# leimao/Voice-Converter-CycleGAN

Measured on NVIDIA H100. Metric: CycleGAN-VC train steps/sec @ batch 256x[24,128] MCEP, higher is better.
Workload: dtype f16f8 (forward / data gradient: fp16 MMA + two e4m3 cross-term MMAs = 2 MMA units per product; weight gradient: fp16 MMA alone, 1 unit; f32 accumulate)

## Files before the change

voice-converter-cyclegan_b200/csrc/tc_gemm.cu:

```cuda
#include "tc_gemm.cuh"
#include "geom.h"
#include "kernels.cuh"
#include "wgmma.cuh"

#include <cuda.h>
#include <stdint.h>
#include <stdio.h>

namespace {

typedef CUresult (*EncodeTiledFn)(CUtensorMap*, CUtensorMapDataType, cuuint32_t, void*, const cuuint64_t*, const cuuint64_t*,
                                  const cuuint32_t*, const cuuint32_t*, CUtensorMapInterleave, CUtensorMapSwizzle,
                                  CUtensorMapL2promotion, CUtensorMapFloatOOBfill);
EncodeTiledFn get_encoder() {
  static EncodeTiledFn fn = nullptr;
  if (!fn) {
    void* p = nullptr; cudaDriverEntryPointQueryResult q;
    if (cudaGetDriverEntryPoint("cuTensorMapEncodeTiled", &p, cudaEnableDefault, &q) == cudaSuccess && q == cudaDriverEntryPointSuccess)
      fn = (EncodeTiledFn)p;
  }
  return fn;
}
bool make_tmap3(CUtensorMap* m, const void* base, uint64_t d0, uint64_t d1, uint64_t d2, uint32_t b1) {
  EncodeTiledFn enc = get_encoder();
  if (!enc) return false;
  cuuint64_t dims[3] = {d0, d1, d2};
  cuuint64_t strides[2] = {d0 * 2, d0 * d1 * 2};
  cuuint32_t box[3] = {64, b1, 1};
  cuuint32_t es[3] = {1, 1, 1};
  return enc(m, CU_TENSOR_MAP_DATA_TYPE_BFLOAT16, 3, const_cast<void*>(base), dims, strides, box, es, CU_TENSOR_MAP_INTERLEAVE_NONE,
             CU_TENSOR_MAP_SWIZZLE_128B, CU_TENSOR_MAP_L2_PROMOTION_L2_256B, CU_TENSOR_MAP_FLOAT_OOB_FILL_NONE) == CUDA_SUCCESS;
}

bool make_tmap3_t(CUtensorMap* m, const void* base, CUtensorMapDataType dt, int esize, uint64_t d0, uint64_t d1, uint64_t d2, uint32_t b0, uint32_t b1) {
  EncodeTiledFn enc = get_encoder();
  if (!enc) return false;
  cuuint64_t dims[3] = {d0, d1, d2};
  cuuint64_t strides[2] = {d0 * (uint64_t)esize, d0 * d1 * (uint64_t)esize};
  cuuint32_t box[3] = {b0, b1, 1};
  cuuint32_t es[3] = {1, 1, 1};
  return enc(m, dt, 3, const_cast<void*>(base), dims, strides, box, es, CU_TENSOR_MAP_INTERLEAVE_NONE,
             b0 * esize == 64 ? CU_TENSOR_MAP_SWIZZLE_64B : CU_TENSOR_MAP_SWIZZLE_128B, CU_TENSOR_MAP_L2_PROMOTION_L2_256B,
             CU_TENSOR_MAP_FLOAT_OOB_FILL_NONE) == CUDA_SUCCESS;
}

__device__ __forceinline__ uint32_t smem_u32(const void* p) { return (uint32_t)__cvta_generic_to_shared(p); }

__device__ __forceinline__ void mbar_init(uint64_t* bar, uint32_t count) {
  asm volatile("mbarrier.init.shared::cta.b64 [%0], %1;" ::"r"(smem_u32(bar)), "r"(count));
}
__device__ __forceinline__ void fence_barrier_init() { asm volatile("fence.mbarrier_init.release.cluster;" ::: "memory"); }
__device__ __forceinline__ void mbar_wait(uint64_t* bar, uint32_t parity) {
  asm volatile(
      "{\n\t"
      ".reg .pred p;\n\t"
      "WAIT_LOOP:\n\t"
      "mbarrier.try_wait.parity.shared::cta.b64 p, [%0], %1;\n\t"
      "@p bra.uni WAIT_DONE;\n\t"
      "bra.uni WAIT_LOOP;\n\t"
      "WAIT_DONE:\n\t"
      "}" ::"r"(smem_u32(bar)), "r"(parity) : "memory");
}
__device__ __forceinline__ void cp_async16(uint32_t dst_smem, const void* src, uint32_t src_bytes) {
  asm volatile("cp.async.cg.shared.global [%0], [%1], 16, %2;" ::"r"(dst_smem), "l"(src), "r"(src_bytes) : "memory");
}
__device__ __forceinline__ void cp_async_arrive_noinc(uint64_t* bar) {
  asm volatile("cp.async.mbarrier.arrive.noinc.shared::cta.b64 [%0];" ::"r"(smem_u32(bar)) : "memory");
}
__device__ __forceinline__ void mbar_expect_tx(uint64_t* bar, uint32_t bytes) {
  asm volatile("mbarrier.arrive.expect_tx.shared::cta.b64 _, [%0], %1;" ::"r"(smem_u32(bar)), "r"(bytes) : "memory");
}
__device__ __forceinline__ void tma_load3(uint32_t dst_smem, const CUtensorMap* map, int c0, int c1, int c2, uint64_t* bar) {
  asm volatile("cp.async.bulk.tensor.3d.shared::cluster.global.tile.mbarrier::complete_tx::bytes [%0], [%1, {%2, %3, %4}], [%5];"
               ::"r"(dst_smem), "l"(map), "r"(c0), "r"(c1), "r"(c2), "r"(smem_u32(bar)) : "memory");
}
__device__ __forceinline__ void tma_prefetch_desc(const CUtensorMap* map) {
  asm volatile("prefetch.tensormap [%0];" ::"l"(map) : "memory");
}
__device__ __forceinline__ void fence_proxy_async() { asm volatile("fence.proxy.async.shared::cta;" ::: "memory"); }
__device__ __forceinline__ uint64_t make_desc(uint32_t smem_addr, uint32_t lbo_bytes, uint32_t sbo_bytes, uint64_t layout = 1) {
  return (uint64_t)((smem_addr >> 4) & 0x3FFF) | ((uint64_t)((lbo_bytes >> 4) & 0x3FFF) << 16) |
         ((uint64_t)((sbo_bytes >> 4) & 0x3FFF) << 32) | (layout << 62);
}
__device__ __forceinline__ uint64_t make_desc64(uint32_t smem_addr) { return make_desc(smem_addr, 16, 512, 2); }
template <int N>
__device__ __forceinline__ void fence_acc(float (&d)[N]) {
#pragma unroll
  for (int i = 0; i < N; ++i) asm volatile("" : "+f"(d[i])::"memory");
}
__device__ __forceinline__ void mbar_arrive(uint64_t* bar) {
  asm volatile("mbarrier.arrive.shared::cta.b64 _, [%0];" ::"r"(smem_u32(bar)) : "memory");
}
__device__ __forceinline__ void consumer_bar() { asm volatile("bar.sync 3, 256;" ::: "memory"); }
__device__ __forceinline__ void st_shared16(uint32_t addr, uint4 v) {
  asm volatile("st.shared.v4.b32 [%0], {%1, %2, %3, %4};" ::"r"(addr), "r"(v.x), "r"(v.y), "r"(v.z), "r"(v.w) : "memory");
}
__device__ __forceinline__ uint4 e4m3x8_to_f16x8(uint2 v) {
  uint32_t w[4];
#pragma unroll
  for (int i = 0; i < 4; ++i) {
    const uint32_t src = (i < 2 ? v.x : v.y) >> (16 * (i & 1));
    const __half2_raw h = __nv_cvt_fp8x2_to_halfraw2((__nv_fp8x2_storage_t)(src & 0xFFFFu), __NV_E4M3);
    w[i] = (uint32_t)h.x | ((uint32_t)h.y << 16);
  }
  return make_uint4(w[0], w[1], w[2], w[3]);
}

struct FastDiv { uint32_t mul, shr, d; };
__host__ inline FastDiv make_fastdiv(uint32_t d) {
  FastDiv f; f.d = d;
  uint32_t l = 0; while ((1ull << l) < d) ++l;
  f.mul = (uint32_t)(((1ull << 32) * ((1ull << l) - d)) / d + 1);
  f.shr = l;
  return f;
}
__device__ __forceinline__ uint32_t fdiv(uint32_t n, const FastDiv& f) { return (uint32_t)(((uint64_t)__umulhi(n, f.mul) + n) >> f.shr); }

__device__ __forceinline__ uint32_t sw128(int r, int c) { return (uint32_t)((r >> 3) * 1024 + (r & 7) * 128 + ((c ^ (r & 7)) << 4)); }

struct TcNTParams {
  GatherGeom g;
  const __nv_bfloat16 *a_hi, *a_lo; int a_ld; int C;
  const __nv_bfloat16 *b_hi, *b_lo; int Nw;
  int N;
  int n_tiles;
  int debug;
  float* dst; int d_ld; const float* bias; int accumulate;
  int perm; int Cc;
  int R;
  const float *gamma_a, *beta_a, *gamma_g, *beta_g;
  float* stats;
  const float* resid;
  float* y; __nv_bfloat16 *y_hi, *y_lo;
  int C_out;
  const float* bp; int bp_ld;
  __nv_bfloat16 *dp_hi, *dp_lo; int dp_ld;
  float *dbeta_a, *dgamma_a, *dbeta_g, *dgamma_g;
  CUtensorMap tm_b_hi, tm_b_lo;
  const uint8_t *a8_hi, *a8_lo;
  CUtensorMap tm_b8_hi, tm_b8_lo;
  uint8_t* y8;
  PackGeom pk;
  FastDiv div_bw, div_w;
};

struct RowPos { int b, y, x; };
__device__ __forceinline__ RowPos nt_row(const TcNTParams& p, long long m) {
  RowPos r;
  r.y = (int)fdiv((uint32_t)m, p.div_bw);
  const uint32_t rem = (uint32_t)m - (uint32_t)r.y * p.div_bw.d;
  r.b = (int)fdiv(rem, p.div_w);
  r.x = (int)(rem - (uint32_t)r.b * p.div_w.d);
  return r;
}
__device__ __forceinline__ uint32_t nt_tile_taps(const TcNTParams& p, long long m0, long long M) {
  const long long m1 = m0 + 127 < M ? m0 + 127 : M - 1;
  return gather_tap_mask(p.g, nt_row(p, m0).y, nt_row(p, m1).y);
}

struct TcTNParams {
  GatherGeom g;
  const __nv_bfloat16 *x_hi, *x_lo; int x_ld; int C;
  const __nv_bfloat16 *g_hi, *g_lo; int g_ld; int N;
  float* dw_a; float* dw_g; int n_split;
  int ksplit;
  FastDiv div_hw, div_w;
  CUtensorMap tm_g_hi, tm_g_lo;
  const uint8_t *x8_hi, *x8_lo;
  const uint8_t *g8_hi, *g8_lo;
  int w16;
  int fold_n;
  float* part; long long part_k, numel_a;
};

__device__ __forceinline__ float* tn_dst(float* base, int slab, int C, int c, int ncols, int col, int fold_n) {
  if (fold_n) { const int t = col / fold_n; return base + ((long long)t * C + c) * fold_n + (col - t * fold_n); }
  return base + ((long long)slab * C + c) * ncols + col;
}

constexpr int kProducerThreads = 128;


template <int BN, int NPL>
struct NTCfg {
  static constexpr int A_PLANE = 128 * 128;
  static constexpr int B_PLANE = BN * 128;
  static constexpr int PLANES = NPL == 2 ? 2 : 1;
  static constexpr int STAGE = PLANES * (A_PLANE + B_PLANE);
  static constexpr int STAGES = (192 * 1024) / STAGE;
  static constexpr int SMEM = STAGES * STAGE + 1024;
  static_assert(STAGES * STAGE >= 128 * BN * 4, "the finished fp32 tile is staged over the pipeline stages");
};

template <int BN>
__device__ __forceinline__ int acc_off(int r, int n) { return r * BN + (n & ~31) + ((((n >> 2) & 7) ^ (r & 7)) << 2) + (n & 3); }
template <int BN>
__device__ __forceinline__ void acc_ld32(const float* acc, int r, int col, uint32_t (&v)[32]) {
#pragma unroll
  for (int c = 0; c < 8; ++c) {
    const float4 x = *reinterpret_cast<const float4*>(acc + r * BN + col + ((c ^ (r & 7)) << 2));
    v[4 * c] = __float_as_uint(x.x); v[4 * c + 1] = __float_as_uint(x.y); v[4 * c + 2] = __float_as_uint(x.z); v[4 * c + 3] = __float_as_uint(x.w);
  }
}

__device__ __forceinline__ float warp_colsum32(float (&t)[32], int lane) {
#pragma unroll
  for (int o = 16, n = 32; o >= 1; o >>= 1, n >>= 1) {
    const bool up = (lane & o) != 0;
#pragma unroll
    for (int i = 0; i < n / 2; ++i) {
      float send = up ? t[i] : t[i + n / 2];
      float keep = up ? t[i + n / 2] : t[i];
      t[i] = keep + __shfl_xor_sync(0xffffffffu, send, o);
    }
  }
  return t[0];
}
__device__ __forceinline__ void epi_bar(int id) { asm volatile("bar.sync %0, 128;" ::"r"(id) : "memory"); }

__device__ __forceinline__ float sample_sum(float v, float (*xch)[32], int q, int lane, int spw, int barid) {
  if (spw == 1) return v;
  epi_bar(barid);
  xch[q][lane] = v;
  epi_bar(barid);
  const int q0 = (q / spw) * spw;
  float r = 0.f;
  for (int w = 0; w < spw; ++w) r += xch[q0 + w][lane];
  return r;
}
__device__ __forceinline__ void bc4(const float* p, float (&v)[4]) { const float4 x = *reinterpret_cast<const float4*>(p); v[0] = x.x; v[1] = x.y; v[2] = x.z; v[3] = x.w; }
__device__ __forceinline__ float fast_sigmoid(float x) { return __fdividef(1.f, 1.f + __expf(-x)); }
__device__ __forceinline__ void chunk_norm_coeffs(const float (&v)[32], const float* __restrict__ gamma, const float* __restrict__ beta,
                                                  int ch, int R, float (*xch)[32], float* bc, int q, int lane, int spw, int barid, float& mean, float& rstd) {
  float t[32];
#pragma unroll
  for (int k = 0; k < 32; ++k) t[k] = v[k];
  float s = warp_colsum32(t, lane);
  s = sample_sum(s, xch, q, lane, spw, barid);
  mean = s / (float)R;
  __syncwarp();
  bc[lane] = mean;
  __syncwarp();
#pragma unroll
  for (int k = 0; k < 32; k += 4) {
    float4 m4 = *reinterpret_cast<const float4*>(bc + k);
    float d0 = v[k] - m4.x, d1 = v[k + 1] - m4.y, d2 = v[k + 2] - m4.z, d3 = v[k + 3] - m4.w;
    t[k] = d0 * d0; t[k + 1] = d1 * d1; t[k + 2] = d2 * d2; t[k + 3] = d3 * d3;
  }
  float ss = warp_colsum32(t, lane);
  ss = sample_sum(ss, xch, q, lane, spw, barid);
  rstd = 1.f / sqrtf(ss / (float)R + 1e-6f);
  const float sc = rstd * gamma[ch + lane];
  const float of = beta[ch + lane] - mean * sc;
  __syncwarp();
  bc[lane] = sc; bc[32 + lane] = of;
  __syncwarp();
}

__device__ __forceinline__ void pair_norm_coeffs(const float (&v0)[32], const float (&v1)[32], const float* __restrict__ gamma, const float* __restrict__ beta,
                                                 int ch, int R, float (*xch)[32], float* bc, int q, int lane, int spw, int barid, float& mean, float& rstd) {
  float t[32];
#pragma unroll
  for (int k = 0; k < 32; ++k) t[k] = v0[k] + v1[k];
  float s = warp_colsum32(t, lane);
  s = sample_sum(s, xch, q, lane, spw, barid);
  const float inv = 1.f / (float)(2 * R);
  mean = s * inv;
  __syncwarp();
  bc[lane] = mean;
  __syncwarp();
#pragma unroll
  for (int k = 0; k < 32; k += 4) {
    float4 m4 = *reinterpret_cast<const float4*>(bc + k);
    const float m[4] = {m4.x, m4.y, m4.z, m4.w};
#pragma unroll
    for (int j = 0; j < 4; ++j) { const float d0 = v0[k + j] - m[j], d1 = v1[k + j] - m[j]; t[k + j] = fmaf(d0, d0, d1 * d1); }
  }
  float ss = warp_colsum32(t, lane);
  ss = sample_sum(ss, xch, q, lane, spw, barid);
  rstd = 1.f / sqrtf(ss * inv + 1e-6f);
  const float sc = rstd * gamma[ch + lane];
  const float of = beta[ch + lane] - mean * sc;
  __syncwarp();
  bc[lane] = sc; bc[32 + lane] = of;
  __syncwarp();
}

__device__ __forceinline__ uint32_t hp_off(int r, int c) { return (uint32_t)(r * 16 + ((c ^ ((r >> 1) & 3)) << 2)); }
template <class F>
__device__ __forceinline__ void rows_out(float* stg, const float (&o)[32], int lane, F f) {
  const int hc = lane & 3, hr = lane >> 2;
#pragma unroll
  for (int h = 0; h < 2; ++h) {
    __syncwarp();
#pragma unroll
    for (int c = 0; c < 4; ++c)
      *reinterpret_cast<float4*>(stg + hp_off(lane, c)) = make_float4(o[16 * h + 4 * c], o[16 * h + 4 * c + 1], o[16 * h + 4 * c + 2], o[16 * h + 4 * c + 3]);
    __syncwarp();
#pragma unroll
    for (int i = 0; i < 4; ++i) {
      const int rr = hr + 8 * i;
      f(rr, 16 * h + 4 * hc, *reinterpret_cast<const float4*>(stg + hp_off(rr, hc)));
    }
  }
}
__device__ __forceinline__ void rows_in(float* stg, float (&v)[32], int lane, const float4 (&pre)[8]) {
  const int hc = lane & 3, hr = lane >> 2;
#pragma unroll
  for (int h = 0; h < 2; ++h) {
    __syncwarp();
#pragma unroll
    for (int i = 0; i < 4; ++i) *reinterpret_cast<float4*>(stg + hp_off(hr + 8 * i, hc)) = pre[4 * h + i];
    __syncwarp();
#pragma unroll
    for (int c = 0; c < 4; ++c) {
      const float4 x = *reinterpret_cast<const float4*>(stg + hp_off(lane, c));
      v[16 * h + 4 * c] = x.x; v[16 * h + 4 * c + 1] = x.y; v[16 * h + 4 * c + 2] = x.z; v[16 * h + 4 * c + 3] = x.w;
    }
  }
}
__device__ __forceinline__ void rows_fetch(float4 (&pre)[8], const float* base, long long ld, long long mq, long long M, int col, int lane) {
  const int hc = lane & 3, hr = lane >> 2;
#pragma unroll
  for (int h = 0; h < 2; ++h)
// ... 598 lines not shown
  static constexpr int SMEM = STAGES * STAGE + 1024;
};

template <int NPL, int W16, int DET>
__global__ void __launch_bounds__(kNTThreads, 1)
tc_gg_tn_kernel(const __grid_constant__ TcTNParams p) {
  static_assert(W16 == 0 || NPL == 3, "the fp16-only weight gradient is a form of CGVC_PREC_F16F8");
  using Cfg = TNCfg<NPL, W16>;
  constexpr int S = Cfg::STAGES;
  constexpr int BN = 256;
  extern __shared__ uint8_t smem_raw[];
  __shared__ __align__(8) uint64_t full_bar[S], empty_bar[S];

  const uint32_t smem_base = (smem_u32(smem_raw) + 1023u) & ~1023u;
  const int warp = threadIdx.x >> 5, lane = threadIdx.x & 31;
  const GatherGeom& g = p.g;
  const long long M = (long long)g.B * g.Hy * g.Wx;
  const int HW = g.Hy * g.Wx;
  const int n_tiles = (p.g_ld + BN - 1) / BN, c_tiles = (p.x_ld + 127) / 128;
  const int num_items = n_tiles * c_tiles * g.ntaps * p.ksplit;
  constexpr int pass0 = (NPL == 3 && !W16) ? 0 : 1;
  long long chunk_rows = (M + p.ksplit - 1) / p.ksplit;
  chunk_rows = (chunk_rows + 63) / 64 * 64;

  struct Item { int n0, c0, tap, ks; long long mbeg, mend; int num_kb; };
  auto decode = [&](int item) -> Item {
    Item w;
    int n_t = item % n_tiles; int t1 = item / n_tiles;
    int c_t = t1 % c_tiles; int t2 = t1 / c_tiles;
    w.tap = t2 % g.ntaps; const int ks = t2 / g.ntaps; w.ks = ks;
    w.n0 = n_t * BN; w.c0 = c_t * 128;
    w.mbeg = (long long)ks * chunk_rows;
    w.mend = (w.mbeg + chunk_rows < M) ? w.mbeg + chunk_rows : M;
    w.num_kb = w.mend > w.mbeg ? (int)((w.mend - w.mbeg + 63) / 64) : 0;
    return w;
  };

  if (threadIdx.x == 0) {
    for (int s = 0; s < S; ++s) { mbar_init(&full_bar[s], kProducerThreads + 1); mbar_init(&empty_bar[s], 8); }
    fence_barrier_init();
    tma_prefetch_desc(&p.tm_g_hi);
    if (NPL == 2) tma_prefetch_desc(&p.tm_g_lo);
  }
  __syncthreads();

  if (warp < 4) {
    const int t = threadIdx.x;
    const int chunk = t & 7, rsub = t >> 3;
    int stage = 0; uint32_t phase = 0;
    for (int item = blockIdx.x; item < num_items; item += gridDim.x) {
      const Item w = decode(item);
      for (int pass = pass0; pass < 2; ++pass)
      for (int kb = 0; kb < w.num_kb; ++kb) {
        mbar_wait(&empty_bar[stage], phase ^ 1);
        const uint32_t sA = smem_base + stage * Cfg::STAGE;
        const uint32_t sB = sA + Cfg::PLANES * Cfg::A_PLANE;
        long long xoff[4];
#pragma unroll
        for (int i = 0; i < 4; ++i) {
          const long long m = w.mbeg + (long long)kb * 64 + rsub + 16 * i;
          xoff[i] = -1;
          if (m < w.mend) {
            const uint32_t mu = (uint32_t)m;
            int b = (int)fdiv(mu, p.div_hw); int rem = (int)(mu - (uint32_t)b * (uint32_t)HW);
            int y = (int)fdiv((uint32_t)rem, p.div_w); int x = rem - y * g.Wx;
            int yy = y * g.sy + g.oy[w.tap], xx = x * g.sx + g.ox[w.tap];
            if (yy >= 0 && yy < g.Hs && xx >= 0 && xx < g.Ws)
              xoff[i] = ((long long)(b * g.Hs + yy) * g.Ws + xx) * p.x_ld + w.c0 + chunk * 8;
          }
        }
        if (NPL == 3 && pass == 0) {
#pragma unroll
          for (int i = 0; i < 4; ++i) {
            const int kr = rsub + 16 * i;
            const uint32_t so = sw128(kr, chunk);
#pragma unroll
            for (int a = 0; a < 2; ++a) {
              const bool ok = xoff[i] >= 0 && (w.c0 + a * 64) < p.x_ld;
              uint2 vh = make_uint2(0u, 0u), vl = make_uint2(0u, 0u);
              if (ok) { vh = __ldg(reinterpret_cast<const uint2*>(p.x8_hi + xoff[i] + a * 64)); vl = __ldg(reinterpret_cast<const uint2*>(p.x8_lo + xoff[i] + a * 64)); }
              st_shared16(sA + a * 8192 + so, e4m3x8_to_f16x8(vh));
              st_shared16(sA + Cfg::A_PLANE + a * 8192 + so, e4m3x8_to_f16x8(vl));
            }
            const long long m = w.mbeg + (long long)kb * 64 + kr;
#pragma unroll
            for (int a = 0; a < 4; ++a) {
              const int col = w.n0 + a * 64 + chunk * 8;
              const bool ok = m < w.mend && col < p.g_ld;
              uint2 vh = make_uint2(0u, 0u), vl = make_uint2(0u, 0u);
              if (ok) { vh = __ldg(reinterpret_cast<const uint2*>(p.g8_hi + m * p.g_ld + col)); vl = __ldg(reinterpret_cast<const uint2*>(p.g8_lo + m * p.g_ld + col)); }
              st_shared16(sB + a * 8192 + so, e4m3x8_to_f16x8(vh));
              st_shared16(sB + Cfg::B_PLANE + a * 8192 + so, e4m3x8_to_f16x8(vl));
            }
          }
          fence_proxy_async();
          if (t == 0) mbar_expect_tx(&full_bar[stage], 0);
          mbar_arrive(&full_bar[stage]);
        } else {
          if (t == 0) {
            const int row0 = (int)(w.mbeg + (long long)kb * 64);
            int natoms = 0;
#pragma unroll
            for (int a = 0; a < 4; ++a) natoms += (w.n0 + a * 64) < p.g_ld ? 1 : 0;
            mbar_expect_tx(&full_bar[stage], (NPL == 2 ? 2 : 1) * natoms * 8192);
#pragma unroll
            for (int a = 0; a < 4; ++a) {
              if ((w.n0 + a * 64) < p.g_ld) {
                tma_load3(sB + a * 8192, &p.tm_g_hi, w.n0 + a * 64, row0, 0, &full_bar[stage]);
                if (NPL == 2) tma_load3(sB + Cfg::B_PLANE + a * 8192, &p.tm_g_lo, w.n0 + a * 64, row0, 0, &full_bar[stage]);
              }
            }
          }
#pragma unroll
          for (int i = 0; i < 4; ++i) {
            const uint32_t so = sw128(rsub + 16 * i, chunk);
#pragma unroll
            for (int a = 0; a < 2; ++a) {
              const bool ok = xoff[i] >= 0 && (w.c0 + a * 64) < p.x_ld;
              const long long off = ok ? xoff[i] + a * 64 : 0;
              cp_async16(sA + a * 8192 + so, p.x_hi + off, ok ? 16u : 0u);
              if (NPL == 2) cp_async16(sA + Cfg::A_PLANE + a * 8192 + so, p.x_lo + off, ok ? 16u : 0u);
            }
          }
          cp_async_arrive_noinc(&full_bar[stage]);
        }
        if (++stage == S) { stage = 0; phase ^= 1; }
      }
    }
  } else {
    const int cw = warp - 4;
    const int wg = cw >> 2;
    const int tw = threadIdx.x - 128 * (wg + 1);
    int stage = 0; uint32_t phase = 0;
    for (int item = blockIdx.x; item < num_items; item += gridDim.x) {
      const Item w = decode(item);
      if (w.num_kb == 0) continue;
      float d[BN / 2];
#pragma unroll
      for (int i = 0; i < BN / 2; ++i) d[i] = 0.f;
      int prev = -1;
      if constexpr (NPL == 3 && !W16) {
        consume_stages<BN, MMA_F16_CROSS, 1, Cfg>(d, w.num_kb, stage, phase, prev, full_bar, empty_bar, smem_base, wg, lane);
        rescale_acc(d, 1.f / (float)(1 << CGVC_Q_WGRAD_SHIFT));
        consume_stages<BN, MMA_F16, 1, Cfg>(d, w.num_kb, stage, phase, prev, full_bar, empty_bar, smem_base, wg, lane);
      } else if constexpr (NPL == 3) {
        consume_stages<BN, MMA_F16, 1, Cfg>(d, w.num_kb, stage, phase, prev, full_bar, empty_bar, smem_base, wg, lane);
      } else {
        consume_stages<BN, NPL == 2 ? MMA_BF16X3 : MMA_BF16, 1, Cfg>(d, w.num_kb, stage, phase, prev, full_bar, empty_bar, smem_base, wg, lane);
      }
      wgmma_wait<0>();
      fence_acc(d);
      if (lane == 0) mbar_arrive(&empty_bar[prev]);
      const int c = w.c0 + wg * 64 + (tw >> 5) * 16 + ((tw & 31) >> 2);
#pragma unroll
      for (int j = 0; j < BN / 8; ++j) {
        const int n = w.n0 + 8 * j + 2 * (tw & 3);
        if (n >= p.N) continue;
        float* base; int nn; int ncols;
        if (n < p.n_split) { base = DET ? p.part + w.ks * p.part_k : p.dw_a; nn = n; ncols = p.n_split; }
        else { base = DET ? p.part + w.ks * p.part_k + p.numel_a : p.dw_g; nn = n - p.n_split; ncols = p.N - p.n_split; }
#pragma unroll
        for (int h = 0; h < 2; ++h) {
          if (c + 8 * h >= p.C) continue;
          float* dst = tn_dst(base, g.widx[w.tap], p.C, c + 8 * h, ncols, nn, p.fold_n);
          if constexpr (DET) asm volatile("st.global.v2.f32 [%0], {%1, %2};" ::"l"(dst), "f"(d[4 * j + 2 * h]), "f"(d[4 * j + 2 * h + 1]) : "memory");
          else asm volatile("red.global.add.v2.f32 [%0], {%1, %2};" ::"l"(dst), "f"(d[4 * j + 2 * h]), "f"(d[4 * j + 2 * h + 1]) : "memory");
        }
      }
    }
  }
}

__host__ __device__ __forceinline__ int perm_row(int perm, int co, int cout, int noff) {
  if (perm == 1) return (co >> 7) * 256 + (noff ? 128 : 0) + (co & 127);
  if (perm == 2) { const int Ch = cout >> 1; const int s = co >= Ch ? 1 : 0; const int c = co - s * Ch; return (c >> 6) * 256 + (noff ? 128 : 0) + s * 64 + (c & 63); }
  return noff + co;
}
__host__ __device__ __forceinline__ long long w_src(int tap, int ci, int co, int cin, int cout, int fold_n) {
  if (fold_n) { const int t = co / fold_n; return ((long long)t * cin + ci) * fold_n + (co - t * fold_n); }
  return ((long long)tap * cin + ci) * cout + co;
}
__global__ void __launch_bounds__(256)
prep_weights_kernel(const float* __restrict__ w, int taps, int cin, int cout, int nt_n, int cin_k, int cin_n, int nt_k, int noff, int perm, int fold_n,
                    __nv_bfloat16* __restrict__ wf_hi, __nv_bfloat16* __restrict__ wf_lo,
                    __nv_bfloat16* __restrict__ wd_hi, __nv_bfloat16* __restrict__ wd_lo) {
  __shared__ float tile[32][33];
  const int tap = blockIdx.z;
  const int ci0 = blockIdx.y * 32, co0 = blockIdx.x * 32;
  const int tx = threadIdx.x & 31, ty = threadIdx.x >> 5;
  for (int r = ty; r < 32; r += 8) {
    int ci = ci0 + r, co = co0 + tx;
    float v = 0.f;
    if (ci < cin && co < cout) {
      v = w[w_src(tap, ci, co, cin, cout, fold_n)];
      __nv_bfloat16 h = __float2bfloat16_rn(v);
      __nv_bfloat16 l = __float2bfloat16_rn(v - __bfloat162float(h));
      long long o = ((long long)tap * cin_n + ci) * nt_k + noff + co;
      wd_hi[o] = h; wd_lo[o] = l;
    }
    tile[r][tx] = v;
  }
  __syncthreads();
  for (int r = ty; r < 32; r += 8) {
    int co = co0 + r, ci = ci0 + tx;
    if (ci < cin && co < cout) {
      float v = tile[tx][r];
      __nv_bfloat16 h = __float2bfloat16_rn(v);
      __nv_bfloat16 l = __float2bfloat16_rn(v - __bfloat162float(h));
      const int nrow = perm_row(perm, co, cout, noff);
      long long o = ((long long)tap * nt_n + nrow) * cin_k + ci;
      wf_hi[o] = h; wf_lo[o] = l;
    }
  }
}

__global__ void copy_bias_kernel(const float* __restrict__ b, float* __restrict__ dst, int n, int noff, int perm) {
  int i = blockIdx.x * 256 + threadIdx.x;
  if (i < n) dst[perm_row(perm, i, n, noff)] = b[i];
}

__global__ void __launch_bounds__(256)
prep_weights_q_kernel(const float* __restrict__ w, int taps, int cin, int cout, int nt_n, int cin_q, int noff, int perm, int fold_n,
                      __half* __restrict__ q16, uint8_t* __restrict__ q8hi, uint8_t* __restrict__ q8lo) {
  const int cq = cin / 4;
  const long long total = (long long)taps * cout * cq;
  for (long long i = (long long)blockIdx.x * 256 + threadIdx.x; i < total; i += (long long)gridDim.x * 256) {
    const int c4 = (int)(i % cq); long long r = i / cq;
    const int co = (int)(r % cout); const int tap = (int)(r / cout);
    const int ci = c4 * 4;
    float v[4];
#pragma unroll
    for (int k = 0; k < 4; ++k) v[k] = w[w_src(tap, ci + k, co, cin, cout, fold_n)];
    const int nrow = perm_row(perm, co, cout, noff);
    const long long o = ((long long)tap * nt_n + nrow) * cin_q + ci;
    uint2 hh; uint32_t b_hi, b_lo;
    cgvc_quant4(v, CGVC_Q_W_SHI, CGVC_Q_W_SLO, hh, b_hi, b_lo);
    *reinterpret_cast<uint2*>(q16 + o) = hh;
    *reinterpret_cast<uint32_t*>(q8hi + o) = b_hi;
    *reinterpret_cast<uint32_t*>(q8lo + o) = b_lo;
  }
}

__global__ void __launch_bounds__(256)
prep_weights_qd_kernel(const float* __restrict__ w, int taps, int cin, int cout, int cin_n, int nt_q, int noff, int fold_n,
                       __half* __restrict__ q16, uint8_t* __restrict__ q8hi, uint8_t* __restrict__ q8lo) {
  const int cq = cout / 4;
  const long long total = (long long)taps * cin * cq;
  for (long long i = (long long)blockIdx.x * 256 + threadIdx.x; i < total; i += (long long)gridDim.x * 256) {
    const int c4 = (int)(i % cq); long long r = i / cq;
    const int ci = (int)(r % cin); const int tap = (int)(r / cin);
    const float4 v4 = *reinterpret_cast<const float4*>(w + w_src(tap, ci, c4 * 4, cin, cout, fold_n));
    const float v[4] = {v4.x, v4.y, v4.z, v4.w};
    const long long o = ((long long)tap * cin_n + ci) * nt_q + noff + c4 * 4;
    uint2 hh; uint32_t b_hi, b_lo;
    cgvc_quant4(v, CGVC_Q_W_SHI, CGVC_Q_W_SLO, hh, b_hi, b_lo);
    *reinterpret_cast<uint2*>(q16 + o) = hh;
    *reinterpret_cast<uint32_t*>(q8hi + o) = b_hi;
    *reinterpret_cast<uint32_t*>(q8lo + o) = b_lo;
  }
}

struct PrepJob {
  long long w_off, b_off;
  int taps, cin, cout, nt_n, cin_q, cin_n, nt_q, noff, perm, fold_n;
  __half* q16; uint8_t *q8hi, *q8lo;
  __half* dq16; uint8_t *dq8hi, *dq8lo;
  float* bias;
  int tiles_ci, tiles_co;
  int first_block;
};

__global__ void __launch_bounds__(256)
prep_weights_q_all_kernel(const float* __restrict__ params, const PrepJob* __restrict__ jobs, int j0, int j1, int block0) {
  __shared__ float tile[32][65];
  const int blk = (int)blockIdx.x + block0;
  int lo = j0, hi = j1 - 1;
  while (lo < hi) { const int mid = (lo + hi + 1) >> 1; if (jobs[mid].first_block <= blk) lo = mid; else hi = mid - 1; }
  const PrepJob& J = jobs[lo];
  int r = blk - J.first_block;
  const int tco = r % J.tiles_co; r /= J.tiles_co;
  const int tci = r % J.tiles_ci; const int tap = r / J.tiles_ci;
  const int ci0 = tci * 32, co0 = tco * 64;
  const float* __restrict__ w = params + J.w_off;
  const int t = threadIdx.x;
  {
    const int c4 = (t & 15) * 4;
    for (int rr = t >> 4; rr < 32; rr += 16) {
      const int ci = ci0 + rr, co = co0 + c4;
      float v[4] = {0.f, 0.f, 0.f, 0.f};
      if (ci < J.cin && co < J.cout) {
        const float4 q = *reinterpret_cast<const float4*>(w + w_src(tap, ci, co, J.cin, J.cout, J.fold_n));
        v[0] = q.x; v[1] = q.y; v[2] = q.z; v[3] = q.w;
        if (J.dq16) {
          const long long o = ((long long)tap * J.cin_n + ci) * J.nt_q + J.noff + co;
          uint2 hh; uint32_t b_hi, b_lo;
          cgvc_quant4(v, CGVC_Q_W_SHI, CGVC_Q_W_SLO, hh, b_hi, b_lo);
          *reinterpret_cast<uint2*>(J.dq16 + o) = hh;
          *reinterpret_cast<uint32_t*>(J.dq8hi + o) = b_hi;
          *reinterpret_cast<uint32_t*>(J.dq8lo + o) = b_lo;
        }
      }
      tile[rr][c4] = v[0]; tile[rr][c4 + 1] = v[1]; tile[rr][c4 + 2] = v[2]; tile[rr][c4 + 3] = v[3];
    }
  }
  __syncthreads();
  {
    const int lane = t & 31, warp = t >> 5;
    const int cig = (lane & 3) * 8;
    const int col = warp * 8 + (lane >> 2);
    const int co = co0 + col;
    if (co < J.cout && ci0 + cig < J.cin_q) {
      float va[4], vb[4];
#pragma unroll
      for (int k = 0; k < 4; ++k) { va[k] = tile[cig + k][col]; vb[k] = tile[cig + 4 + k][col]; }
      const int nrow = perm_row(J.perm, co, J.cout, J.noff);
      const long long o = ((long long)tap * J.nt_n + nrow) * J.cin_q + ci0 + cig;
      uint2 ha, hb; uint32_t a_hi, a_lo, b_hi, b_lo;
      cgvc_quant4(va, CGVC_Q_W_SHI, CGVC_Q_W_SLO, ha, a_hi, a_lo);
      cgvc_quant4(vb, CGVC_Q_W_SHI, CGVC_Q_W_SLO, hb, b_hi, b_lo);
      *reinterpret_cast<uint4*>(J.q16 + o) = make_uint4(ha.x, ha.y, hb.x, hb.y);
      *reinterpret_cast<uint2*>(J.q8hi + o) = make_uint2(a_hi, b_hi);
      *reinterpret_cast<uint2*>(J.q8lo + o) = make_uint2(a_lo, b_lo);
    }
  }
  if (tap == 0 && tci == 0 && tco == 0 && J.b_off >= 0)
    for (int i = t; i < J.cout; i += 256) J.bias[perm_row(J.perm, i, J.cout, J.noff)] = params[J.b_off + i];
}

template <class K>
cudaError_t set_smem(K kernel, int bytes) {
  static std::vector<const void*> done;
  const void* key = (const void*)kernel;
  for (const void* d : done) if (d == key) return cudaSuccess;
  cudaError_t e = cudaFuncSetAttribute(kernel, cudaFuncAttributeMaxDynamicSharedMemorySize, bytes);
  if (e == cudaSuccess) done.push_back(key);
  return e;
}

struct ProfRec { cudaEvent_t a, b; double flops; int cls; long long M; int N, K; };
int g_tc_debug = 0;
int g_tc_prep_batched = 1;
bool g_prof_on = false;
std::vector<ProfRec> g_prof;
void prof_begin(cudaStream_t st, double flops, int cls, long long M = 0, int N = 0, int K = 0) {
  if (!g_prof_on) return;
  ProfRec r; r.flops = flops; r.cls = cls; r.M = M; r.N = N; r.K = K;
  cudaEventCreate(&r.a); cudaEventCreate(&r.b);
  cudaEventRecord(r.a, st);
  g_prof.push_back(r);
}
void prof_end(cudaStream_t st) { if (g_prof_on && !g_prof.empty()) cudaEventRecord(g_prof.back().b, st); }

inline int tile_rows(int n_real, int n_padded) { return (n_padded % 256 == 0) ? 256 : (n_real <= 32 ? 32 : 128); }

int num_sms() {
  static int n = 0;
  if (!n) { int dev = 0; cudaGetDevice(&dev); cudaDeviceGetAttribute(&n, cudaDevAttrMultiProcessorCount, dev); }
  return n;
}

cudaError_t launch_nt(TcNTParams p, int precision, cudaStream_t st, int epi) {
  const long long M = (long long)p.g.B * p.g.Hy * p.g.Wx;
  if (M == 0) return cudaSuccess;
  if (M >= (1ll << 31)) return cudaErrorInvalidValue;
  const bool x3 = precision == 1;
  if (p.g.ntaps == 0) return cudaErrorInvalidValue;
  p.div_bw = make_fastdiv((uint32_t)(p.g.B * p.g.Wx)); p.div_w = make_fastdiv((uint32_t)p.g.Wx);
  const int bn = tile_rows(p.N, p.Nw);
  p.n_tiles = bn == 32 ? 1 : p.Nw / bn;
  const long long tiles = ((M + 127) / 128) * p.n_tiles;
  dim3 grid((unsigned)(tiles < num_sms() ? tiles : num_sms()));
  cudaError_t e;
  ++g_cgvc_launches;
  p.debug = g_tc_debug;
  prof_begin(st, 2.0 * (double)M * p.N * p.g.ntaps * p.C, (epi == 1 || epi == 2 || epi == 5) ? 2 : 0, M, p.N, p.g.ntaps * p.C);
#define LAUNCH_NT(BN_, NPL_, EPI_, ...)                                                                        \
  do {                                                                                                         \
    e = set_smem(tc_gg_nt_kernel<BN_, NPL_, EPI_, ##__VA_ARGS__>, NTCfg<BN_, NPL_>::SMEM);                     \
    if (e != cudaSuccess) return e;                                                                            \
    tc_gg_nt_kernel<BN_, NPL_, EPI_, ##__VA_ARGS__><<<grid, kNTThreads, NTCfg<BN_, NPL_>::SMEM, st>>>(p);      \
  } while (0)
  if (epi != 0 && bn != 256) return cudaErrorInvalidValue;
  if (p.pk.off) {
    if (epi != 0 || p.g.B != 1 || p.g.Hy != 1) return cudaErrorInvalidValue;
    const int npl = precision == 3 ? 3 : x3 ? 2 : 1;
    if (bn == 256)      { if (npl == 3) LAUNCH_NT(256, 3, 0, true); else if (npl == 2) LAUNCH_NT(256, 2, 0, true); else LAUNCH_NT(256, 1, 0, true); }
    else if (bn == 128) { if (npl == 3) LAUNCH_NT(128, 3, 0, true); else if (npl == 2) LAUNCH_NT(128, 2, 0, true); else LAUNCH_NT(128, 1, 0, true); }
    else                { if (npl == 3) LAUNCH_NT(32, 3, 0, true);  else if (npl == 2) LAUNCH_NT(32, 2, 0, true);  else LAUNCH_NT(32, 1, 0, true); }
  }
  else if (precision == 3) {
    if (epi == 1)       LAUNCH_NT(256, 3, 1);
    else if (epi == 2)  LAUNCH_NT(256, 3, 2);
    else if (epi == 5)  LAUNCH_NT(256, 3, 5);
    else if (epi != 0)  return cudaErrorInvalidValue;
    else if (bn == 256) LAUNCH_NT(256, 3, 0);
    else if (bn == 128) LAUNCH_NT(128, 3, 0);
    else                LAUNCH_NT(32, 3, 0);
  }
  else if (epi == 1)  { if (x3) LAUNCH_NT(256, 2, 1); else LAUNCH_NT(256, 1, 1); }
  else if (epi == 2)  { if (x3) LAUNCH_NT(256, 2, 2); else LAUNCH_NT(256, 1, 2); }
  else if (epi == 3)  { if (x3) LAUNCH_NT(256, 2, 3); else LAUNCH_NT(256, 1, 3); }
  else if (epi == 4)  { if (x3) LAUNCH_NT(256, 2, 4); else LAUNCH_NT(256, 1, 4); }
  else if (epi == 5)  { if (x3) LAUNCH_NT(256, 2, 5); else LAUNCH_NT(256, 1, 5); }
  else if (bn == 256) { if (x3) LAUNCH_NT(256, 2, 0); else LAUNCH_NT(256, 1, 0); }
  else if (bn == 128) { if (x3) LAUNCH_NT(128, 2, 0); else LAUNCH_NT(128, 1, 0); }
  else                { if (x3) LAUNCH_NT(32, 2, 0);  else LAUNCH_NT(32, 1, 0); }
#undef LAUNCH_NT
  prof_end(st);
  return cudaGetLastError();
}

cudaError_t launch_tn(TcTNParams p, int precision, cudaStream_t st, const DetSlab* det) {
  const long long M = (long long)p.g.B * p.g.Hy * p.g.Wx;
  if (M == 0) return cudaSuccess;
  if (M >= (1ll << 31)) return cudaErrorInvalidValue;
  const int tiles = ((p.g_ld + 255) / 256) * ((p.x_ld + 127) / 128) * p.g.ntaps;
  const int nsm = num_sms();
  long long maxsplit = M / 1024; if (maxsplit < 1) maxsplit = 1; if (maxsplit > 32) maxsplit = 32;
  int ksplit = 1; double best = 0.0;
  for (int ks = 1; ks <= (int)maxsplit; ++ks) {
    long long items = (long long)tiles * ks;
    double eff = (double)items / (double)(((items + nsm - 1) / nsm) * nsm);
    if (items < nsm) eff *= 0.5;
    if (eff > best + 0.02) { best = eff; ksplit = ks; }
  }
  const long long numel = (long long)p.g.ntaps * p.C * p.N;
  auto chunk_of = [&](int ks) { return ((M + ks - 1) / ks + 63) / 64 * 64; };
  if (det && det->p)
    while (ksplit > 1 && ((long long)ksplit * numel > det->cap || (long long)(ksplit - 1) * chunk_of(ksplit) >= M)) --ksplit;
  const bool det_split = det && det->p && ksplit > 1;
  if (det_split) { p.part = det->p; p.part_k = numel; p.numel_a = (long long)p.g.ntaps * p.C * p.n_split; }
  p.ksplit = ksplit;
  p.div_hw = make_fastdiv((uint32_t)(p.g.Hy * p.g.Wx)); p.div_w = make_fastdiv((uint32_t)p.g.Wx);
  const long long items = (long long)tiles * ksplit;
  dim3 grid((unsigned)(items < nsm ? items : nsm));
  cudaError_t e;
  ++g_cgvc_launches;
  prof_begin(st, 2.0 * (double)M * p.N * p.g.ntaps * p.C, 1, M, p.N, p.g.ntaps * p.C);
#define LAUNCH_TN(NPL_, W16_, DET_)                                                               \
  do {                                                                                            \
    e = set_smem(tc_gg_tn_kernel<NPL_, W16_, DET_>, TNCfg<NPL_, W16_>::SMEM);                     \
    if (e != cudaSuccess) return e;                                                               \
    tc_gg_tn_kernel<NPL_, W16_, DET_><<<grid, kNTThreads, TNCfg<NPL_, W16_>::SMEM, st>>>(p);      \
  } while (0)
  if (det_split) {
    if (precision == 3) { if (p.w16) LAUNCH_TN(3, 1, 1); else LAUNCH_TN(3, 0, 1); }
    else if (precision == 1) LAUNCH_TN(2, 0, 1);
    else                     LAUNCH_TN(1, 0, 1);
  } else {
    if (precision == 3) { if (p.w16) LAUNCH_TN(3, 1, 0); else LAUNCH_TN(3, 0, 0); }
    else if (precision == 1) LAUNCH_TN(2, 0, 0);
    else                     LAUNCH_TN(1, 0, 0);
  }
#undef LAUNCH_TN
  prof_end(st);
  if (!det_split) return cudaGetLastError();
  e = cudaGetLastError();
  if (e != cudaSuccess) return e;
  return launch_reduce_parts(p.part, ksplit, numel, DetSegs{{p.dw_a, p.dw_g}, {0, p.numel_a}, {p.numel_a, p.dw_g ? numel - p.numel_a : 0}}, st);
}

inline int ru(int v, int m) { return (v + m - 1) / m * m; }
inline int Ntot(const TcLayer& L) { return L.cout * (L.gated ? 2 : 1); }
inline int cin_k(const TcLayer& L) { return ru(L.cin, 64); }
inline int cin_n(const TcLayer& L) { return ru(L.cin, 128); }
inline int nt_k(const TcLayer& L) { return ru(Ntot(L), 64); }
inline int nt_n(const TcLayer& L) { return ru(Ntot(L), 128); }
inline int cin_q(const TcLayer& L) { return ru(L.cin, 128); }
inline int nt_q(const TcLayer& L) { return ru(Ntot(L), 128); }
inline size_t wq_elems(const TcLayer& L) { return (size_t)L.kh * L.kw * nt_n(L) * cin_q(L); }
inline size_t wdq_elems(const TcLayer& L) { return (size_t)L.kh * L.kw * cin_n(L) * nt_q(L); }
inline size_t wf_elems(const TcLayer& L) { return (size_t)L.kh * L.kw * nt_n(L) * cin_k(L); }
inline size_t wd_elems(const TcLayer& L) { return (size_t)L.kh * L.kw * cin_n(L) * nt_k(L); }
inline int layer_perm(const TcLayer& L) {
  if (L.gated && L.shuffle == 2 && L.cout % 128 == 0) return 2;
  return (L.gated && L.cout % 128 == 0) ? 1 : 0;
}
inline bool layer_ok(const TcLayer& L) {
  if (L.fold && (L.gated || L.kh * L.kw != 1 || L.cout % L.fold || (L.cout / L.fold) % 4)) return false;
  return L.kh * L.kw <= CGVC_MAX_TAPS && Ntot(L) % 4 == 0;
}
inline bool layer_ok_q(const TcLayer& L) { return layer_ok(L) && L.cin % 4 == 0; }


bool make_layer_maps(TcLayer& L) {
  const int taps = L.kh * L.kw;
  const int bf = tile_rows(Ntot(L), nt_n(L)), bd = tile_rows(L.cin, cin_n(L));
  return make_tmap3(&L.tm_f_hi, L.wf_hi, cin_k(L), nt_n(L), taps, bf) &&
         make_tmap3(&L.tm_f_lo, L.wf_lo, cin_k(L), nt_n(L), taps, bf) &&
         make_tmap3(&L.tm_d_hi, L.wd_hi, nt_k(L), cin_n(L), taps, bd) &&
         make_tmap3(&L.tm_d_lo, L.wd_lo, nt_k(L), cin_n(L), taps, bd);
}

bool make_layer_maps_q(TcLayer& L) {
  const int taps = L.kh * L.kw;
  const int bf = tile_rows(Ntot(L), nt_n(L)), bd = tile_rows(L.cin, cin_n(L));
  const CUtensorMapDataType F16 = CU_TENSOR_MAP_DATA_TYPE_FLOAT16, U8 = CU_TENSOR_MAP_DATA_TYPE_UINT8;
  bool ok = make_tmap3_t(&L.tm_q16, L.wq16, F16, 2, cin_q(L), nt_n(L), taps, 64, bf) &&
            make_tmap3_t(&L.tm_q8hi, L.wq8hi, U8, 1, cin_q(L), nt_n(L), taps, 64, bf) &&
            make_tmap3_t(&L.tm_q8lo, L.wq8lo, U8, 1, cin_q(L), nt_n(L), taps, 64, bf);
  if (ok && L.wdq16)
    ok = make_tmap3_t(&L.tm_dq16, L.wdq16, F16, 2, nt_q(L), cin_n(L), taps, 64, bd) &&
         make_tmap3_t(&L.tm_dq8hi, L.wdq8hi, U8, 1, nt_q(L), cin_n(L), taps, 64, bd) &&
         make_tmap3_t(&L.tm_dq8lo, L.wdq8lo, U8, 1, nt_q(L), cin_n(L), taps, 64, bd);
  return ok;
}


int refresh_layer(TcLayer& L, const float* ka, const float* kg, const float* ba, const float* bg, cudaStream_t st) {
  const int taps = L.kh * L.kw;
  dim3 grid((L.cout + 31) / 32, (L.cin + 31) / 32, taps);
  g_cgvc_launches += L.gated ? 4 : 2;
  const int perm = layer_perm(L);
  const int fn = L.fold ? L.cout / L.fold : 0;
  if (!L.wq16) prep_weights_kernel<<<grid, 256, 0, st>>>(ka, taps, L.cin, L.cout, nt_n(L), cin_k(L), cin_n(L), nt_k(L), 0, perm, fn, L.wf_hi, L.wf_lo, L.wd_hi, L.wd_lo);
  if (!L.fold) copy_bias_kernel<<<(L.cout + 255) / 256, 256, 0, st>>>(ba, L.bias, L.cout, 0, perm);
  if (L.gated) {
    if (!L.wq16) prep_weights_kernel<<<grid, 256, 0, st>>>(kg, taps, L.cin, L.cout, nt_n(L), cin_k(L), cin_n(L), nt_k(L), L.cout, perm, fn, L.wf_hi, L.wf_lo, L.wd_hi, L.wd_lo);
    copy_bias_kernel<<<(L.cout + 255) / 256, 256, 0, st>>>(bg, L.bias, L.cout, L.cout, perm);
  }
  if (L.wq16) {
    long long tot = (long long)taps * L.cout * (L.cin / 4); long long nb = (tot + 255) / 256; if (nb > num_sms() * 32) nb = num_sms() * 32;
    g_cgvc_launches += L.gated ? 2 : 1;
    prep_weights_q_kernel<<<(unsigned)nb, 256, 0, st>>>(ka, taps, L.cin, L.cout, nt_n(L), cin_q(L), 0, perm, fn, (__half*)L.wq16, L.wq8hi, L.wq8lo);
    if (L.gated) prep_weights_q_kernel<<<(unsigned)nb, 256, 0, st>>>(kg, taps, L.cin, L.cout, nt_n(L), cin_q(L), L.cout, perm, fn, (__half*)L.wq16, L.wq8hi, L.wq8lo);
    if (L.wdq16) {
      g_cgvc_launches += L.gated ? 2 : 1;
      prep_weights_qd_kernel<<<(unsigned)nb, 256, 0, st>>>(ka, taps, L.cin, L.cout, cin_n(L), nt_q(L), 0, fn, (__half*)L.wdq16, L.wdq8hi, L.wdq8lo);
      if (L.gated) prep_weights_qd_kernel<<<(unsigned)nb, 256, 0, st>>>(kg, taps, L.cin, L.cout, cin_n(L), nt_q(L), L.cout, fn, (__half*)L.wdq16, L.wdq8hi, L.wdq8lo);
    }
  }
  return (int)cudaGetLastError();
}

int layer_fwd(const TcLayer& L, int precision, const __nv_bfloat16* xhi, const __nv_bfloat16* xlo, int n, int H, int W, int sh, int sw,
              float* P, cudaStream_t st, const TcFuse* fuse = nullptr, bool* fused_out = nullptr, const PackGeom* pk = nullptr) {
  if (!layer_ok(L) || (precision == 3 && !layer_ok_q(L))) return TC_UNSUPPORTED;
  if (pk && (n != 1 || H != 1 || L.kh != 1 || fuse)) return (int)cudaErrorInvalidValue;
  TcNTParams p; memset(&p, 0, sizeof p);
  p.g = fwd_geom(n, H, W, L.kh, L.kw, sh, sw);
  if (pk) p.pk = *pk;
  p.a_hi = xhi; p.a_lo = xlo; p.a_ld = cin_k(L); p.C = cin_k(L);
  p.b_hi = L.wf_hi; p.b_lo = L.wf_lo; p.Nw = nt_n(L); p.N = Ntot(L);
  p.dst = P; p.d_ld = Ntot(L); p.bias = L.bias; p.accumulate = 0;
  p.perm = layer_perm(L); p.Cc = L.cout;
  p.tm_b_hi = L.tm_f_hi; p.tm_b_lo = L.tm_f_lo;
  if (precision == 3) {
    if (!L.wq16) return TC_UNSUPPORTED;
    p.a_ld = cin_q(L); p.C = cin_q(L); p.a_lo = nullptr;
    p.a8_hi = reinterpret_cast<const uint8_t*>(xlo); p.a8_lo = p.a8_hi + (size_t)n * H * W * cin_q(L);
    p.tm_b_hi = L.tm_q16; p.tm_b8_hi = L.tm_q8hi; p.tm_b8_lo = L.tm_q8lo;
  }
  int epi = 0;
  if (fuse && fuse->R > 0) {
    const bool shape_ok = H == 1 && (fuse->R == 32 || fuse->R == 64 || fuse->R == 128) && p.g.Wx == fuse->R && nt_n(L) % 256 == 0 && Ntot(L) == nt_n(L);
    if (shape_ok && L.gated && p.perm == 1) epi = 1; else if (shape_ok && L.gated && p.perm == 2) epi = 5; else if (shape_ok && !L.gated) epi = 2;
    if (epi) {
      p.R = fuse->R; p.gamma_a = fuse->gamma_a; p.beta_a = fuse->beta_a; p.gamma_g = fuse->gamma_g; p.beta_g = fuse->beta_g;
      p.stats = fuse->stats; p.resid = fuse->resid; p.y = fuse->y; p.y_hi = fuse->y_hi; p.y_lo = fuse->y_lo;
      p.y8 = reinterpret_cast<uint8_t*>(fuse->y_lo);
      p.C_out = epi == 5 ? L.cout / 2 : (L.gated ? L.cout : Ntot(L));
      if (!p.y_hi || (epi == 2 && !p.resid)) epi = 0;
    }
  }
  if (fused_out) *fused_out = epi != 0;
  if (!epi && !P) return (int)cudaErrorInvalidValue;
  return (int)launch_nt(p, precision, st, epi);
}

int layer_dgrad(const TcLayer& L, int precision, const __nv_bfloat16* dPhi, const __nv_bfloat16* dPlo, int n, int H, int W, int sh, int sw,
                float* dx, int accumulate, cudaStream_t st, const TcBwdFuse* fuse = nullptr, bool* fused_out = nullptr) {
  if (fused_out) *fused_out = false;
  if (!layer_ok(L) || (precision == 3 && (!layer_ok_q(L) || !L.wdq16))) return TC_UNSUPPORTED;
  std::vector<GatherGeom> gs = dgrad_geoms(n, H, W, L.kh, L.kw, sh, sw);
  for (const GatherGeom& g : gs) if (g.ntaps == 0) return TC_UNSUPPORTED;
  int epi = 0;
  if (fuse && fuse->R > 0 && gs.size() == 1 && H == 1 && sh == 1 && sw == 1 && (fuse->R == 32 || fuse->R == 64 || fuse->R == 128) &&
      gs[0].Wx == fuse->R && cin_n(L) % 256 == 0 && L.cin == cin_n(L) && fuse->bp && fuse->stats && fuse->dp_hi && fuse->dp_lo && fuse->gamma_a &&
      (fuse->gated ? (fuse->gamma_g && fuse->beta_a && fuse->beta_g) : (dx != nullptr)) && precision != 3)
    epi = fuse->gated ? 3 : 4;
  for (const GatherGeom& g : gs) {
    TcNTParams p; memset(&p, 0, sizeof p);
    p.g = g;
    p.a_hi = dPhi; p.a_lo = dPlo; p.a_ld = nt_k(L); p.C = nt_k(L);
    p.b_hi = L.wd_hi; p.b_lo = L.wd_lo; p.Nw = cin_n(L); p.N = L.cin;
// ... 327 lines not shown
```

Before: 9.984.

## Pick weight-grad K-split by modeled makespan and vectorize epilogue stores

Two changes to the weight-gradient (TN) GEMM. The split-K selection heuristic now simulates the per-CTA work, counting chunk passes plus a fixed flush cost and handling tail chunks, and picks the split with the smallest worst-case CTA time. The old rule maximized wave efficiency instead. The epilogue gains a 'quad' mode that swaps accumulator halves between lane pairs with shuffles, so each thread issues one 16-byte v4 store or red.add instead of two 8-byte v2 ones. This halves the atomic/store instruction count, at the cost of shuffles and an alignment/divisibility check that falls back to the old path.

```diff
diff --git a/voice-converter-cyclegan_b200/csrc/tc_gemm.cu b/voice-converter-cyclegan_b200/csrc/tc_gemm.cu
--- a/voice-converter-cyclegan_b200/csrc/tc_gemm.cu
+++ b/voice-converter-cyclegan_b200/csrc/tc_gemm.cu
@@ -170,6 +170,7 @@
   const uint8_t *g8_hi, *g8_lo;
   int w16;
   int fold_n;
+  int quad;
   float* part; long long part_k, numel_a;
 };
 
@@ -1074,19 +1075,39 @@
       fence_acc(d);
       if (lane == 0) mbar_arrive(&empty_bar[prev]);
       const int c = w.c0 + wg * 64 + (tw >> 5) * 16 + ((tw & 31) >> 2);
-#pragma unroll
-      for (int j = 0; j < BN / 8; ++j) {
-        const int n = w.n0 + 8 * j + 2 * (tw & 3);
-        if (n >= p.N) continue;
+      auto dst_of = [&](int row, int n) {
         float* base; int nn; int ncols;
         if (n < p.n_split) { base = DET ? p.part + w.ks * p.part_k : p.dw_a; nn = n; ncols = p.n_split; }
         else { base = DET ? p.part + w.ks * p.part_k + p.numel_a : p.dw_g; nn = n - p.n_split; ncols = p.N - p.n_split; }
-#pragma unroll
-        for (int h = 0; h < 2; ++h) {
-          if (c + 8 * h >= p.C) continue;
-          float* dst = tn_dst(base, g.widx[w.tap], p.C, c + 8 * h, ncols, nn, p.fold_n);
-          if constexpr (DET) asm volatile("st.global.v2.f32 [%0], {%1, %2};" ::"l"(dst), "f"(d[4 * j + 2 * h]), "f"(d[4 * j + 2 * h + 1]) : "memory");
-          else asm volatile("red.global.add.v2.f32 [%0], {%1, %2};" ::"l"(dst), "f"(d[4 * j + 2 * h]), "f"(d[4 * j + 2 * h + 1]) : "memory");
+        return tn_dst(base, g.widx[w.tap], p.C, row, ncols, nn, p.fold_n);
+      };
+      if (p.quad) {
+        const bool odd = tw & 1;
+        const int row = c + (odd ? 8 : 0);
+#pragma unroll
+        for (int j = 0; j < BN / 8; ++j) {
+          const float r0 = __shfl_xor_sync(0xffffffffu, odd ? d[4 * j] : d[4 * j + 2], 1);
+          const float r1 = __shfl_xor_sync(0xffffffffu, odd ? d[4 * j + 1] : d[4 * j + 3], 1);
+          const float v0 = odd ? r0 : d[4 * j], v1 = odd ? r1 : d[4 * j + 1];
+          const float v2 = odd ? d[4 * j + 2] : r0, v3 = odd ? d[4 * j + 3] : r1;
+          const int n = w.n0 + 8 * j + 4 * ((tw & 3) >> 1);
+          if (n >= p.N || row >= p.C) continue;
+          float* dst = dst_of(row, n);
+          if constexpr (DET) asm volatile("st.global.v4.f32 [%0], {%1, %2, %3, %4};" ::"l"(dst), "f"(v0), "f"(v1), "f"(v2), "f"(v3) : "memory");
+          else asm volatile("red.global.add.v4.f32 [%0], {%1, %2, %3, %4};" ::"l"(dst), "f"(v0), "f"(v1), "f"(v2), "f"(v3) : "memory");
+        }
+      } else {
+#pragma unroll
+        for (int j = 0; j < BN / 8; ++j) {
+          const int n = w.n0 + 8 * j + 2 * (tw & 3);
+          if (n >= p.N) continue;
+#pragma unroll
+          for (int h = 0; h < 2; ++h) {
+            if (c + 8 * h >= p.C) continue;
+            float* dst = dst_of(c + 8 * h, n);
+            if constexpr (DET) asm volatile("st.global.v2.f32 [%0], {%1, %2};" ::"l"(dst), "f"(d[4 * j + 2 * h]), "f"(d[4 * j + 2 * h + 1]) : "memory");
+            else asm volatile("red.global.add.v2.f32 [%0], {%1, %2};" ::"l"(dst), "f"(d[4 * j + 2 * h]), "f"(d[4 * j + 2 * h + 1]) : "memory");
+          }
         }
       }
     }
@@ -1332,27 +1353,45 @@
   return cudaGetLastError();
 }
 
+constexpr double kTNFlushStages = 4.0;
+
+inline long long tn_chunk_rows(long long M, int ks) { return ((M + ks - 1) / ks + 63) / 64 * 64; }
+
+inline double tn_split_cost(long long M, int tiles, int ks, int nsm, int passes) {
+  const long long chunk = tn_chunk_rows(M, ks);
+  const long long items = (long long)tiles * ks, grid = items < nsm ? items : nsm;
+  const long long nfull = M / chunk, tail = M - nfull * chunk;
+  const long long a = nfull * tiles, b = a + (tail ? tiles : 0);
+  const double c_full = (double)(chunk / 64 * passes) + kTNFlushStages, c_tail = (double)((tail + 63) / 64 * passes) + kTNFlushStages;
+  auto count = [&](long long x, long long j) { return x > j ? (x - j + grid - 1) / grid : 0; };
+  double worst = 0.0;
+  for (long long j = 0; j < grid; ++j) {
+    const double c = (double)count(a, j) * c_full + (double)(count(b, j) - count(a, j)) * c_tail;
+    if (c > worst) worst = c;
+  }
+  return worst;
+}
+
 cudaError_t launch_tn(TcTNParams p, int precision, cudaStream_t st, const DetSlab* det) {
   const long long M = (long long)p.g.B * p.g.Hy * p.g.Wx;
   if (M == 0) return cudaSuccess;
   if (M >= (1ll << 31)) return cudaErrorInvalidValue;
   const int tiles = ((p.g_ld + 255) / 256) * ((p.x_ld + 127) / 128) * p.g.ntaps;
   const int nsm = num_sms();
+  const long long numel = (long long)p.g.ntaps * p.C * p.N;
+  const bool det_on = det && det->p;
   long long maxsplit = M / 1024; if (maxsplit < 1) maxsplit = 1; if (maxsplit > 32) maxsplit = 32;
-  int ksplit = 1; double best = 0.0;
+  int ksplit = 1; double best = -1.0;
   for (int ks = 1; ks <= (int)maxsplit; ++ks) {
-    long long items = (long long)tiles * ks;
-    double eff = (double)items / (double)(((items + nsm - 1) / nsm) * nsm);
-    if (items < nsm) eff *= 0.5;
-    if (eff > best + 0.02) { best = eff; ksplit = ks; }
-  }
-  const long long numel = (long long)p.g.ntaps * p.C * p.N;
-  auto chunk_of = [&](int ks) { return ((M + ks - 1) / ks + 63) / 64 * 64; };
-  if (det && det->p)
-    while (ksplit > 1 && ((long long)ksplit * numel > det->cap || (long long)(ksplit - 1) * chunk_of(ksplit) >= M)) --ksplit;
-  const bool det_split = det && det->p && ksplit > 1;
+    if (det_on && ks > 1 && ((long long)ks * numel > det->cap || (long long)(ks - 1) * tn_chunk_rows(M, ks) >= M)) continue;
+    const double c = tn_split_cost(M, tiles, ks, nsm, (precision == 3 && !p.w16) ? 2 : 1);
+    if (best < 0.0 || c < best) { best = c; ksplit = ks; }
+  }
+  const bool det_split = det_on && ksplit > 1;
   if (det_split) { p.part = det->p; p.part_k = numel; p.numel_a = (long long)p.g.ntaps * p.C * p.n_split; }
   p.ksplit = ksplit;
+  auto al16 = [](const void* q) { return ((uintptr_t)q & 15) == 0; };
+  p.quad = (p.N % 4 == 0 && p.n_split % 4 == 0 && p.fold_n % 4 == 0 && (det_split ? al16(p.part) : al16(p.dw_a) && al16(p.dw_g))) ? 1 : 0;
   p.div_hw = make_fastdiv((uint32_t)(p.g.Hy * p.g.Wx)); p.div_w = make_fastdiv((uint32_t)p.g.Wx);
   const long long items = (long long)tiles * ksplit;
   dim3 grid((unsigned)(items < nsm ? items : nsm));
```

Result: no change. 10.08 (median of 6 runs) (+1.0%).
